# Ajay-Wong/seq2seq-attention-asr

Hardware: AMD Instinct MI355X
Metric: log-mel frames/sec fwd+bwd, Chorowski TIMIT baseline (higher is better)
Workload: dtype fp32; 1 GPU; BASELINE config 2: timit_chorowski_b32; model=timit/model_chorowski_baseline.lua, global_batch=32, utterances_per_gpu=32, seq_len=128, label_len=40, feat_dim=123, parallelism=dp1, allreduce=none, launch=hipGraph replay

## Files before the change

### seq2seq-attention-asr_amd/csrc/gru_persist.hip

```cpp
#include <algorithm>
#include <cstdlib>

#include "gru.h"
#include "gru_persist.h"
#include "handoff.h"
#include "skinny.h"

namespace s2s {

namespace {

struct PDir {
  const float* xp;
  long ldxp;
  const float* Wa;
  const float* Wb;
  float* y;
  long ldy;
  float* sv;
  const float* dy;
  long lddy;
  float* dA;
  long ldA;
  int reverse;
// ... 47 lines not shown
  x.ct = rem - x.d * q.ntn;
  return x;
}
__device__ __forceinline__ bool xunit_of(const XProj& q, int nd, int p, int nprod, int it, XUnit& x) {
  const int w = p + it * nprod;
  if (q.G == 0 || w < q.nsplit) {
    if (w >= q.nwork) return false;
    x = xunit(q, nd, w);
    return true;
  }
  const int nsp = q.nsplit > p ? (q.nsplit - p + nprod - 1) / nprod : 0;
  const int g = p / q.gsz, v = p - g * q.gsz + (it - nsp) * q.gsz;
  const int ncls = q.G / nd, i = v / q.ntn;
  x.sl = q.sB + i * ncls + g / nd;
  if (x.sl >= q.nslices) return false;
  x.d = g % nd;
  x.ct = v - i * q.ntn;
  x.part = 0;
  x.P = 1;
  x.item = -1;
  return true;
}
constexpr int kXpLds = 4 * 64 * 36 * 4;

struct WArgs {
  int nw;
  float* dW[2][3];
  float scale;
  const float* x;
  long ldx;
  int D, NP;
  float* part;
  unsigned* ticket;
  unsigned long long* stamps;
};

struct PArgs {
  XProj xq;
  int fused;
  PDir d[2];
  int B, L, H, MT, nwg;
  int nmem, nchains;
  int allow_local;
  unsigned* abort_word;
  unsigned* census;
  const int* len;
  char* next_sync;
  size_t next_prep;
  GruPackJobs pack;
  int ring;
  int stream_sweep;
  unsigned long long* stamps;
  unsigned long long* pstamps;
  int prefetch, prefetch_wg;
  unsigned* progress;
  WArgs wg;
};

#ifndef S2S_GRU_DIAG
#define S2S_GRU_DIAG 0
#endif
constexpr int kStampSlots = S2S_GRU_DIAG ? 16 : 8;
#define GRU_STAMP(ph)                                                                      \
  do {                                                                                     \
    if (a.stamps && threadIdx.x == 0)                                                      \
      a.stamps[((long)lw * a.L + s) * kStampSlots + (ph)] = __builtin_amdgcn_s_memrealtime(); \
  } while (0)
#define GRU_STAMP_V(ph, v)                                                                 \
  do {                                                                                     \
    if (a.stamps && threadIdx.x == 0) a.stamps[((long)lw * a.L + s) * kStampSlots + (ph)] = (v); \
  } while (0)
#if S2S_GRU_DIAG
template <int NC>
__device__ __forceinline__ bool sweep_sent_n(float4 (&a)[NC], __amdgpu_buffer_rsrc_t rs, long tbase, int rowt,
                                             int wave, int lane, unsigned* abort_word, unsigned& n) {
  const long lo = tbase + 4 * tile_lane(rowt, lane);
  unsigned spins = 0;
  while (true) {
    ++n;
    bool ok = true;
#pragma unroll
    for (int i = 0; i < NC; ++i) {
      const long off = lo + 4L * 256 * (wave + 4 * i);
      const uint4 p = __builtin_bit_cast(uint4, __builtin_amdgcn_raw_buffer_load_b128(rs, (int)off, 0, 16));
      ok = ok && p.x != kSent && p.y != kSent && p.z != kSent && p.w != kSent;
      a[i] = make_float4(__uint_as_float(p.x), __uint_as_float(p.y), __uint_as_float(p.z), __uint_as_float(p.w));
    }
    if (__all(ok)) return true;
    if (spin_give_up(spins, abort_word)) return false;
  }
}
#define SWEEP_SENT(slot_, ...) sweep_sent_n<NC>(__VA_ARGS__, npoll[slot_])
#else
#define SWEEP_SENT(slot_, ...) sweep_sent_tile<NC>(__VA_ARGS__)
#endif
std::atomic<unsigned long long*> g_gru_stamps[2] = {{nullptr}, {nullptr}};
std::atomic<unsigned long long*> g_gru_pstamps[2] = {{nullptr}, {nullptr}};
std::atomic<unsigned long long*> g_gru_wstamps{nullptr};
constexpr int kProdStampItems = 32;

__device__ __forceinline__ float reduce_or_abort(SkinnyRed& red, int* abort_lds, bool ok, floatx4 acc, int wave,
                                                 int lane, int tid, bool* aborted) {
  if (!ok) *abort_lds = 1;
  const float s = skinny_reduce(red, acc, wave, lane, tid);
  *aborted = *abort_lds != 0;
  return s;
}

template <bool NN, int D>
__device__ __forceinline__ void xproj_produce(const PArgs& a, float* lds, int p, int nprod) {
  const XProj& q = a.xq;
  const int tid = threadIdx.x, lane = tid & 63, wave = tid >> 6;
  const int nk = q.K / 32;
  __shared__ int last_part;
  const int nd = q.nd;
  if (tid >= 256) {
    XUnit x;
    for (int it = 0; xunit_of(q, nd, p, nprod, it, x); ++it) {
      const int nb = 1 + nk / x.P + (q.alpha ? 1 : 0);
      for (int i = 0; i < nb; ++i) __syncthreads();
      if (x.P == 1) {
        __syncthreads();
      } else {
        __syncthreads();
        __syncthreads();
        if (last_part) __syncthreads();
      }
    }
    return;
  }
  const int wy = wave >> 1, wx = wave & 1, li = lane & 31, lk = lane >> 5;
  const int B = a.B, L = a.L, H3 = q.ncd;
  constexpr int LDK = 36;
  float* As[2] = {lds, lds + 64 * LDK};
  float* Bs[2] = {lds + 128 * LDK, lds + 192 * LDK};
  int item = 0;
  XUnit xu;
  for (; xunit_of(q, nd, p, nprod, item, xu); ++item) {
    if (a.pstamps && tid == 0 && item < kProdStampItems)
      a.pstamps[((long)p * kProdStampItems + item) * 2] = __builtin_amdgcn_s_memrealtime();
    const int sl = xu.sl, d = xu.d, ct = xu.ct;
    const int nkp = nk / xu.P, kb = xu.part * nkp;
    const int rev = a.d[d].reverse ^ q.flip;
    const float* arow[2];
    const float* brow[2];
#pragma unroll
    for (int j = 0; j < 2; ++j) {
      const int r = (tid >> 3) + 32 * j, jt = r / B, b = r - jt * B, s = sl * q.tpt + jt;
      const bool aval = jt < q.tpt && s < L;
      const int t = rev ? L - 1 - s : s;
      arow[j] = q.x + (aval ? ((long)b * L + t) * q.ldx : 0);
      const int f = tid + 256 * j;
      brow[j] = NN ? q.W + (long)(f & 31) * q.ldw + d * H3 + ct * 64 + 4 * (f >> 5)
                   : q.W + (long)(d * H3 + ct * 64 + r) * q.ldw;
    }
    const int kq = 4 * (tid & 7);
    const long bstep = NN ? 32 * q.ldw : 32;
    floatx4 ra[D][2], rb[D][2];
    auto gload = [&](floatx4 (&xa)[2], floatx4 (&xb)[2], int kt) {
#pragma unroll
      for (int j = 0; j < 2; ++j) {
        xa[j] = *reinterpret_cast<const floatx4*>(arow[j] + 32 * kt + kq);
        xb[j] = *reinterpret_cast<const floatx4*>(brow[j] + kt * bstep + (NN ? 0 : kq));
      }
    };
    auto lstore = [&](const floatx4 (&xa)[2], const floatx4 (&xb)[2], int buf) {
      float* as = As[0] + buf * (64 * LDK);
      float* bs = Bs[0] + buf * (64 * LDK);
#pragma unroll
      for (int j = 0; j < 2; ++j) {
        const int f = tid + 256 * j;
        *reinterpret_cast<floatx4*>(as + (f >> 3) * LDK + 4 * (f & 7)) = xa[j];
        if (NN) {
          float* pb = bs + (4 * (f >> 5)) * LDK + (f & 31);
          pb[0] = xb[j][0];
          pb[LDK] = xb[j][1];
          pb[2 * LDK] = xb[j][2];
          pb[3 * LDK] = xb[j][3];
        } else {
          *reinterpret_cast<floatx4*>(bs + (f >> 3) * LDK + 4 * (f & 7)) = xb[j];
        }
      }
    };
    floatx16 acc;
#pragma unroll
    for (int r = 0; r < 16; ++r) acc[r] = 0.f;
    auto mma = [&](int buf, auto&& mid) {
      floatx4 av[4], bv[4];
      const float* pa = As[0] + buf * (64 * LDK) + (wy * 32 + li) * LDK + 16 * lk;
      const float* pb = Bs[0] + buf * (64 * LDK) + (wx * 32 + li) * LDK + 16 * lk;
#pragma unroll
// ... 110 lines not shown
        for (int i = 0; i < 4; ++i)
          pv[pp][i] = pp < xu.P ? __builtin_bit_cast(floatx4, __builtin_amdgcn_raw_buffer_load_b128(
                                                                  srs, ibase + pp * 16384 + 16 * i, 0, 16))
                                : floatx4{0.f, 0.f, 0.f, 0.f};
#pragma unroll
      for (int i = 0; i < 4; ++i)
#pragma unroll
        for (int e = 0; e < 4; ++e) {
          float v = pv[0][i][e] + pv[1][i][e];
          if (xu.P > 2) v = (v + pv[2][i][e]) + pv[3][i][e];
          acc[4 * i + e] = v;
        }
    }
#pragma unroll
    for (int r = 0; r < 16; ++r) {
      const int tr = wy * 32 + (r & 3) + 8 * (r >> 2) + 4 * lk, jt = tr / B, b = tr - jt * B, s = sl * q.tpt + jt;
      if (jt < q.tpt && s < L) {
        const int t = rev ? L - 1 - s : s;
        __hip_atomic_store(q.xp + ((long)b * L + t) * q.ldxp + col, 1.f * acc[r], __ATOMIC_RELAXED,
                           __HIP_MEMORY_SCOPE_AGENT);
      }
    }
    asm volatile("s_waitcnt vmcnt(0)" ::: "memory");
    __syncthreads();
    if (tid == 0) __hip_atomic_fetch_add(q.done + d * q.nslices + sl, 1u, __ATOMIC_RELAXED, __HIP_MEMORY_SCOPE_AGENT);
    if (a.pstamps && tid == 0 && item < kProdStampItems)
      a.pstamps[((long)p * kProdStampItems + item) * 2 + 1] = __builtin_amdgcn_s_memrealtime();
  }
}

template <bool NN>
__device__ __forceinline__ void xproj_produce_any(const PArgs& a, float* lds, int p, int nprod) {
  const int nk = a.xq.K / 32;
  if (nk % 4 == 0) xproj_produce<NN, 4>(a, lds, p, nprod);
  else if (nk % 3 == 0) xproj_produce<NN, 3>(a, lds, p, nprod);
  else if (nk % 2 == 0) xproj_produce<NN, 2>(a, lds, p, nprod);
  else xproj_produce<NN, 1>(a, lds, p, nprod);
}

__device__ __forceinline__ bool xproj_ready(const XProj& q, int d, int sl) {
  return __hip_atomic_load(q.done + d * q.nslices + sl, __ATOMIC_RELAXED, __HIP_MEMORY_SCOPE_AGENT) >=
         (unsigned)q.ntn;
}

__device__ __forceinline__ void xproj_wait(const XProj& q, int d, int need, int& ready, int lane, unsigned* abort_word) {
  unsigned spins = 0;
  while (need >= ready) {
    const int sl = ready + lane;
    const unsigned long long nr = __ballot(!(sl >= q.nslices || xproj_ready(q, d, sl)));
    const int upto = nr ? ready + (int)__builtin_ctzll(nr) : ready + 64;
    if (upto <= need && spin_give_up(spins, abort_word)) break;
    ready = upto;
  }
}

__device__ __forceinline__ void prep_next_sync(const PArgs& a, int sp, int nsp) {
  if (!a.next_sync) return;
  if (sp == 0 && threadIdx.x == 0) {
    unsigned* hdr = reinterpret_cast<unsigned*>(a.next_sync);
    const unsigned e = __hip_atomic_fetch_add(&g_s2s_epoch_ctr, 1u, __ATOMIC_RELAXED, __HIP_MEMORY_SCOPE_AGENT) + 1u;
    __hip_atomic_exchange(hdr + kEpochWord, e, __ATOMIC_RELAXED, __HIP_MEMORY_SCOPE_AGENT);
    rearm_abort_word(hdr);
  }
  const size_t n16 = (a.next_prep - 256) / 16;
  uint4* p = reinterpret_cast<uint4*>(a.next_sync + 256);
  for (size_t i = (size_t)sp * blockDim.x + threadIdx.x; i < n16; i += (size_t)nsp * blockDim.x)
    p[i] = make_uint4(0u, 0u, 0u, 0u);
  if (threadIdx.x == 0 && sp == 0 && (a.next_prep - 256) % 16) {
    unsigned* t = reinterpret_cast<unsigned*>(a.next_sync + 256 + n16 * 16);
    for (size_t i = 0; i < ((a.next_prep - 256) % 16) / 4; ++i) t[i] = 0u;
  }
}

constexpr int kRowRing = 4;
constexpr int kSentRing = 4;
__device__ __forceinline__ int sent_slot(const PArgs& a, int s) { return a.ring ? (s & (a.ring - 1)) : s; }
__device__ __forceinline__ void rearm_tile(float* role, const PArgs& a, int s, long tile, int lane) {
  const float4 sv = make_float4(__uint_as_float(kSent), __uint_as_float(kSent), __uint_as_float(kSent),
                                __uint_as_float(kSent));
  *reinterpret_cast<float4*>(role + (long)sent_slot(a, s) * a.MT * 16 * a.H + tile + 4 * lane) = sv;
}
constexpr int kFwdThreads = 320;
template <int NC>
__global__ __launch_bounds__(kFwdThreads) void gru_fwd_persist(PArgs a) {
  __shared__ SkinnyRed red;
  __shared__ int abort_lds, local_lds;
  __shared__ unsigned tb_lds;
  __shared__ __attribute__((aligned(16))) float hprev[16][16];
  __shared__ __attribute__((aligned(16))) float xring[kRowRing][2][256];
  __shared__ __attribute__((aligned(16))) float stg[2][3][256];
  extern __shared__ __attribute__((aligned(16))) float xlds[];
  const int H = a.H, B = a.B, L = a.L;
  const ChainSlot cs = chain_slot(a.nmem);
  if (cs.chain >= a.nchains) {
    const int gch = 8 * ((a.nchains + 7) / 8);
    const int sp = (cs.chain - a.nchains) * a.nmem + cs.member, nsp = (gch - a.nchains) * a.nmem;
    prep_next_sync(a, sp, nsp);
    if (a.fused) xproj_produce_any<false>(a, xlds, sp, nsp);
    for (int j = 0; j < a.pack.n; ++j)
      gru_pack_elems(a.pack.j[j], (long)sp * blockDim.x + threadIdx.x, (long)nsp * blockDim.x);
    return;
  }
  const int dir = cs.chain / a.MT, mt = cs.chain % a.MT;
  const PDir& g = a.d[dir];
  const int ncol = 2 * H / 16;
  const int c1 = cs.member;
  const int lw = dir * a.nwg + mt * ncol + c1;
  const bool isz = c1 < H / 16;
  const int tid = threadIdx.x, lane = tid & 63, wave = tid >> 6;
  const int b0 = mt * 16;
  if (tid == 0) abort_lds = 0;
  const unsigned tb = launch_tagbase(a.abort_word, &tb_lds);
  const bool loader = wave == 4;
  const long mytile = (long)mt * 16 * H + (long)(isz ? c1 : c1 - H / 16) * 256;
  if (!loader)
    rearm_rect((isz ? g.s0 : g.s1) + mytile, (long)a.MT * 16 * H, a.ring ? a.ring : L, 16, 0, 16, 0, 16);
  rearm_done();
  const bool loc = chain_is_local(a.census, cs.chain, a.nmem, c1, a.allow_local != 0, a.abort_word, &local_lds, tb);

  if (loader) {
    const int bl = b0 + (lane >> 2), col = c1 * 16 + 4 * (lane & 3);
    const bool lv = bl < B;
    const __amdgpu_buffer_rsrc_t xr = rsrc_of(g.xp);
    int xready = 0;
    auto issue = [&](int q, float4 (&r)[2]) {
      r[0] = r[1] = make_float4(0.f, 0.f, 0.f, 0.f);
      if (q >= L) return;
      if (a.fused) xproj_wait(a.xq, dir, q / a.xq.tpt, xready, lane, a.abort_word);
      if (!lv) return;
      const int t = g.reverse ? L - 1 - q : q;
      const long off = ((long)bl * L + t) * g.ldxp + col;
      if (a.fused) {
        r[0] = __builtin_bit_cast(float4, __builtin_amdgcn_raw_buffer_load_b128(xr, (int)(4 * off), 0, 16));
        if (isz)
          r[1] = __builtin_bit_cast(float4, __builtin_amdgcn_raw_buffer_load_b128(xr, (int)(4 * (off + 2 * H)), 0, 16));
      } else {
        r[0] = *reinterpret_cast<const float4*>(g.xp + off);
        if (isz) r[1] = *reinterpret_cast<const float4*>(g.xp + off + 2 * H);
      }
    };
    auto put = [&](int q, const float4 (&r)[2]) {
      *reinterpret_cast<float4*>(&xring[q % kRowRing][0][4 * lane]) = r[0];
      *reinterpret_cast<float4*>(&xring[q % kRowRing][1][4 * lane]) = r[1];
    };
    auto store = [&](int q) {
      if (!lv) return;
      const int t = g.reverse ? L - 1 - q : q;
      const long row = (long)bl * L + t;
      const float4 v0 = *reinterpret_cast<const float4*>(&stg[q & 1][0][4 * lane]);
      const float4 v1 = *reinterpret_cast<const float4*>(&stg[q & 1][1][4 * lane]);
      const float4 v2 = *reinterpret_cast<const float4*>(&stg[q & 1][2][4 * lane]);
      float* sv = g.sv + row * 5 * H;
      if (isz) {
        *reinterpret_cast<float4*>(sv + col) = v0;
        *reinterpret_cast<float4*>(sv + 2 * H + col) = v1;
        *reinterpret_cast<float4*>(g.y + row * g.ldy + col) = v2;
      } else {
        const int j = col - H;
        *reinterpret_cast<float4*>(sv + H + j) = v0;
        *reinterpret_cast<float4*>(sv + 3 * H + j) = v1;
        *reinterpret_cast<float4*>(sv + 4 * H + j) = v2;
      }
    };
    float4 ra[2], rb[2];
    issue(0, ra);
    issue(1, rb);
    put(0, ra);
    put(1, rb);
    issue(2, ra);
    __syncthreads();
    const bool ring = a.ring && loc;
    for (int s = 0; s < L; ++s) {
      if (ring) asm volatile("s_waitcnt vmcnt(0)" ::: "memory");
      __syncthreads();
      if (abort_lds) return;
      if (s > 0) store(s - 1);
      put(s + 2, ra);
      issue(s + 3, ra);
      if (ring) {
        if (isz && s >= 2) rearm_tile(g.s0, a, s - 2, mytile, lane);
        if (!isz && s >= 1) rearm_tile(g.s1, a, s - 1, mytile, lane);
      }
      if (!isz) continue;
      __syncthreads();
      if (abort_lds) return;
    }
    __syncthreads();
    store(L - 1);
    return;
  }

  float4 w1[NC], w2[NC];
  load_wfrag(w1, g.Wa + (long)(c1 * 16 + (lane & 15)) * H, wave, lane);
  if (isz) load_wfrag(w2, g.Wb + (long)(c1 * 16 + (lane & 15)) * H, wave, lane);

  const __amdgpu_buffer_rsrc_t hg = rsrc_of(g.g0), qg = rsrc_of(g.g1), hs = rsrc_of(g.s0), qs = rsrc_of(g.s1);
  const long slot = (long)B * H;
  const long slotS = (long)a.MT * 16 * H, tileS = (long)mt * 16 * H;
  const int rowt = min(b0 + (lane & 15), B - 1) - b0;
  const int br = min(b0 + (lane & 15), B - 1);
  const int ob = b0 + (tid >> 4), on = c1 * 16 + (tid & 15);
  const bool live = ob < B;
  const int lenb = (a.len && live) ? a.len[ob] : L;
  const int jt = c1 * 16 - H, wt = (jt % 64) / 16, it = jt / 64;
  float zreg = 0.f, hreg = 0.f;
  bool aborted = false;

  __syncthreads();
  for (int s = 0; s < L; ++s) {
    const int t = g.reverse ? L - 1 - s : s;
    floatx4 acc = {0.f, 0.f, 0.f, 0.f};
    bool ok = true;
    GRU_STAMP(0);
    if (s > 0) {
      float4 av[NC];
#if S2S_GRU_DIAG
      unsigned npoll[1] = {0};
#endif
      {
      if (loc) ok = SWEEP_SENT(0, av, hs, 4 * (sent_slot(a, s - 1) * slotS + tileS), rowt, wave, lane, a.abort_word);
      else ok = sweep_skinny<NC>(av, hg, 8 * (((s - 1) & 1) * slot + (long)br * H), tb + s, wave, lane, a.abort_word);
      GRU_STAMP(1);
#if S2S_GRU_DIAG
      GRU_STAMP_V(8, npoll[0]);
#endif
      acc = mfma_chunks<NC>(av, w1);
      }
      if (!isz && wave == wt) {
#pragma unroll
        for (int i = 0; i < NC; ++i)
          if (i == it) *reinterpret_cast<float4*>(&hprev[lane & 15][4 * (lane >> 4)]) = av[i];
// ... 315 lines not shown
  __shared__ int abort_lds, local_lds;
  __shared__ unsigned tb_lds;
  __shared__ __attribute__((aligned(16))) float rowq[kRowRing][5][256];
  extern __shared__ __attribute__((aligned(16))) float ylds[];
  const int H = a.H, B = a.B, L = a.L;
  const ChainSlot cs = chain_slot(a.nmem);
  const int gch = 8 * ((a.nchains + 7) / 8);
  if ((int)blockIdx.x >= chain_grid(a.nchains, a.nmem)) {
    const int pre = chain_grid(a.nchains, a.nmem) + (a.prefetch ? 8 * a.prefetch_wg : 0);
    if ((int)blockIdx.x < pre) {
      const int e = (int)blockIdx.x - chain_grid(a.nchains, a.nmem), c = e & 7, w = e >> 3;
      if (c < a.nchains) bptt_prefetch<NC>(a, c, w, a.prefetch_wg);
      return;
    }
    const int e = (int)blockIdx.x - pre, c = e & 7, w = e >> 3;
    if (c < a.nchains) bptt_wgrad<NC>(a, c, w, &tb_lds, &abort_lds);
    return;
  }
  if (cs.chain >= a.nchains) {
    const int sp = (cs.chain - a.nchains) * a.nmem + cs.member, nsp = (gch - a.nchains) * a.nmem;
    prep_next_sync(a, sp, nsp);
    if (a.fused) xproj_produce_any<true>(a, ylds, sp, nsp);
    return;
  }
  const int dir = cs.chain / a.MT, mt = cs.chain % a.MT;
  const PDir& g = a.d[dir];
  const int ncol = H / 16;
  const int c = cs.member;
  const int lw = dir * a.nwg + mt * ncol + c;
  const int tid = threadIdx.x, lane = tid & 63, wave = tid >> 6;
  const int b0 = mt * 16;
  if (a.stamps && tid == 0) a.stamps[((long)lw * L + L - 1) * 8 + 6] = __builtin_amdgcn_s_memrealtime();
  if (tid == 0) abort_lds = 0;
  const unsigned tb = launch_tagbase(a.abort_word, &tb_lds);
  const bool loader = wave == 4;
  const long mytile = (long)mt * 16 * H + (long)c * 256;
  if (!loader) {
    const long st = (long)a.MT * 16 * H;
    const int ns = a.ring ? a.ring : L;
    rearm_rect(g.s0 + mytile, st, ns, 16, 0, 16, 0, 16);
    rearm_rect(g.s1 + mytile, st, ns, 16, 0, 16, 0, 16);
    rearm_rect(g.s2 + mytile, st, ns, 16, 0, 16, 0, 16);
  }
  rearm_done();
  const bool loc = chain_is_local(a.census, cs.chain, a.nmem, c, a.allow_local != 0, a.abort_word, &local_lds, tb);
  if (a.stamps && tid == 0) a.stamps[((long)lw * L + L - 1) * 8 + 7] = __builtin_amdgcn_s_memrealtime();

  if (loader) {
    const int bl = b0 + (lane >> 2), u = c * 16 + 4 * (lane & 3);
    const bool lv = bl < B;
    const int lenl = (a.len && lv) ? a.len[bl] : L;
    const __amdgpu_buffer_rsrc_t dyr = rsrc_of(g.dy);
    int yready = 0;
    auto issue = [&](int q, float4 (&r)[5]) {
#pragma unroll
      for (int v = 0; v < 5; ++v) r[v] = make_float4(0.f, 0.f, 0.f, 0.f);
      if (q >= L) return;
      if (a.fused) xproj_wait(a.xq, dir, q / a.xq.tpt, yready, lane, a.abort_word);
      if (!lv) return;
#ifdef S2S_EXP_NOLOAD
      return;
#endif
      const int t = g.reverse ? q : L - 1 - q;
      const long row = (long)bl * L + t;
      const float* sv = g.sv + row * 5 * H + u;
#pragma unroll
      for (int v = 0; v < 4; ++v) r[v] = *reinterpret_cast<const float4*>(sv + v * H);
      if (t >= lenl) return;
      if (a.fused) {
        r[4] = __builtin_bit_cast(float4, __builtin_amdgcn_raw_buffer_load_b128(
                                              dyr, (int)(4 * (row * g.lddy + u)), 0, 16));
      } else {
        r[4] = *reinterpret_cast<const float4*>(g.dy + row * g.lddy + u);
      }
    };
    auto put = [&](int q, const float4 (&r)[5]) {
#pragma unroll
      for (int v = 0; v < 5; ++v) *reinterpret_cast<float4*>(&rowq[q % kRowRing][v][4 * lane]) = r[v];
    };
    float4 ra[5], rb[5];
    issue(0, ra);
    issue(1, rb);
    put(0, ra);
    put(1, rb);
    issue(2, ra);
    __syncthreads();
    const bool ring = a.ring && loc;
    unsigned* prog = a.progress ? a.progress + (long)cs.chain * a.nmem + c : nullptr;
    for (int p = 0; p < L; ++p) {
      __syncthreads();
      if (abort_lds) return;
      put(p + 2, ra);
      if (prog && lane == 0) __hip_atomic_store(prog, (unsigned)p, __ATOMIC_RELAXED, __HIP_MEMORY_SCOPE_WORKGROUP);
#ifndef S2S_EXP_LOADB
      issue(p + 3, ra);
#endif
      if (ring && p >= 1) {
        rearm_tile(g.s0, a, p - 1, mytile, lane);
        rearm_tile(g.s1, a, p - 1, mytile, lane);
        rearm_tile(g.s2, a, p - 1, mytile, lane);
      }
      asm volatile("s_waitcnt vmcnt(0)" ::: "memory");
      __syncthreads();
      if (abort_lds) return;
#ifdef S2S_EXP_LOADB
      issue(p + 3, ra);
#endif
    }
    if (a.wg.nw) {
      __syncthreads();
      if (lane == 0) __hip_atomic_store(prog, (unsigned)L + 3u, __ATOMIC_RELAXED, __HIP_MEMORY_SCOPE_AGENT);
    }
    return;
  }

  float4 wh[NC], wzr[2 * NC];
  load_wfrag(wh, g.Wa + (long)(c * 16 + (lane & 15)) * H, wave, lane);
  load_wfrag(wzr, g.Wb + (long)(c * 16 + (lane & 15)) * 2 * H, wave, lane);
  const __amdgpu_buffer_rsrc_t zg = rsrc_of(g.g0), rg = rsrc_of(g.g1), hg = rsrc_of(g.g2);
  const __amdgpu_buffer_rsrc_t zs = rsrc_of(g.s0), rs_ = rsrc_of(g.s1), hs = rsrc_of(g.s2);
  const long slot = (long)B * H;
  const int br = min(b0 + (lane & 15), B - 1);
  const long slotS = (long)a.MT * 16 * H, tileS = (long)mt * 16 * H;
  const int rowt = br - b0;
  const int ob = b0 + (tid >> 4), ok_ = c * 16 + (tid & 15);
  const bool live = ob < B;
  const int lenb = (a.len && live) ? a.len[ob] : L;
  float dhc = 0.f, dhp = 0.f;
  bool aborted = false;

  struct Row {
    float z, r, hh, hp, dy;
  };
  auto load_row = [&](int q) {
    const float(*r)[256] = rowq[q % kRowRing];
    return Row{r[0][tid], r[1][tid], r[2][tid], r[3][tid], r[4][tid]};
  };
  auto gate = [&](int t, const Row& v, float dh, int pn, bool pub) {
    const long row = (long)ob * L + t;
    const float daz = dh * (v.hh - v.hp) * (v.z * (1.0f - v.z));
    const float dah = (dh * v.z) * (1.0f - v.hh * v.hh);
    if (loc) {
      const long off = sent_slot(a, pn) * slotS + tile_off(ob, ok_, H);
      if (pub) {
        put_sent(g.s2 + off, dah);
        put_sent(g.s0 + off, daz);
      }
    } else {
      const long off = (pn & 1) * slot + (long)ob * H + ok_;
      put_granule_pair(g.g2, off, dah, tb + pn + 1, pub);
      put_granule_pair(g.g0, off, daz, tb + pn + 1, pub);
    }
#ifndef S2S_EXP_NODA
    if (pub) {
      g.dA[row * g.ldA + ok_] = daz;
      g.dA[row * g.ldA + 2 * H + ok_] = dah;
    }
#endif
  };

// ... 120 lines not shown
  const int nch = ndir * ((B + 15) / 16), nm = H / 16;
  const int nwg = std::max(1, std::min((int)g_bptt_prefetch_wg, nm));
  return g_bptt_prefetch > 0 && nch <= 8 && nm + nwg <= 32 && nm % nwg == 0 ? nwg : 0;
}
std::atomic<int> g_allow_local{1};
std::atomic<int> g_sent_ring{kSentRing};
std::atomic<int> g_stream_sweep{1};

template <int NC>
int launch_nc(hipStream_t st, const PArgs& a, bool excl_req, bool fwd) {
  const dim3 grid(chain_grid(a.nchains, a.nmem) + (!fwd && a.prefetch ? 8 * a.prefetch_wg : 0) +
                  (!fwd ? 8 * a.wg.nw : 0));
  const bool excl = excl_req && a.nchains <= 8 && a.nmem <= 32;
  const unsigned shm = excl ? kExclLds : (a.fused ? kXpLds : 0);
  if (fwd) {
    if (excl) S2S_CHECK_HIP(hipFuncSetAttribute(reinterpret_cast<const void*>(gru_fwd_persist<NC>),
                                                hipFuncAttributeMaxDynamicSharedMemorySize, kExclLds));
    S2S_TRY(check_resident(reinterpret_cast<const void*>(gru_fwd_persist<NC>), grid.x, kFwdThreads, shm,
                           "gru_fwd_persist"));
    hipLaunchKernelGGL(gru_fwd_persist<NC>, grid, dim3(kFwdThreads), shm, st, a);
  } else {
    if (excl) S2S_CHECK_HIP(hipFuncSetAttribute(reinterpret_cast<const void*>(gru_bwd_persist<NC>),
                                                hipFuncAttributeMaxDynamicSharedMemorySize, kExclLds));
    S2S_TRY(check_resident(reinterpret_cast<const void*>(gru_bwd_persist<NC>), grid.x, kBwdThreads, shm,
                           "gru_bwd_persist"));
    hipLaunchKernelGGL(gru_bwd_persist<NC>, grid, dim3(kBwdThreads), shm, st, a);
  }
  S2S_CHECK_HIP(hipGetLastError());
  return 0;
}

int launch(hipStream_t st, const PArgs& a, bool excl, bool fwd) {
  switch (a.H / 64) {
    case 1: return launch_nc<1>(st, a, excl, fwd);
    case 2: return launch_nc<2>(st, a, excl, fwd);
    case 4: return launch_nc<4>(st, a, excl, fwd);
    case 8: return launch_nc<8>(st, a, excl, fwd);
  }
  set_error("gru persistent: unsupported H");
  return 2;
}

}

std::atomic<int> g_fuse_xproj{1};

bool gru_persist_fused_xproj(int ndir, int B, int H, int Kx) {
  if (!g_fuse_xproj || B > 64 || Kx % 32 != 0 || H % 64 != 0) return false;
  const int MT = (B + 15) / 16, nchains = ndir * MT, nmem = 2 * H / 16;
  return chain_grid(nchains, nmem) - nchains * nmem >= 32;
}

std::atomic<int> g_xp_split{1};
std::atomic<int> g_fuse_dy{1};

bool gru_persist_fused_dy(int ndir, int B, int H, int K, long ldw, long lddy) {
  if (!g_fuse_xproj || !g_fuse_dy || B > 64 || K % 32 != 0 || H % 64 != 0 || ldw % 4 != 0 || lddy < (long)ndir * H) return false;
  const int MT = (B + 15) / 16, nchains = ndir * MT, nmem = H / 16;
  return chain_grid(nchains, nmem) - nchains * nmem >= 32;
}

bool gru_persist_wgrad_fits(int ndir, int B, int H, int D) {
  const int nch = ndir * ((B + 15) / 16), nm = H / 16, nw = 3 * H / 64;
  return H % 64 == 0 && D > 0 && nch <= 8 && nm + bptt_prefetch_wg(ndir, B, H) + nw <= 32 &&
         H + (D + 15) / 16 * 16 <= 4 * kWgCB * 16;
}

bool gru_persist_supported(int ndir, int B, int H) {
  if (!(H == 64 || H == 128 || H == 256 || H == 512)) return false;
  const int MT = (B + 15) / 16;
  return (2 * H / 16) * ((ndir * MT + 7) / 8) <= 64;
}

static size_t census_bytes(int B, int H) { return 4 * (size_t)(2 * ((B + 15) / 16)) * (2 * H / 16); }

static size_t xcount_words(int L) { return 2 * (size_t)L + kXpMaxSplitItems; }
static size_t prep_bytes(int B, int L, int H) {
  return 256 + 2 * 3 * 2 * sizeof(unsigned long long) * (size_t)B * H + census_bytes(B, H) + 4 * xcount_words(L) +
         census_bytes(B, H);
}
static size_t sent_offset(int B, int L, int H) { return (prep_bytes(B, L, H) + 255) / 256 * 256; }
static size_t sent_rows(int B) { return (size_t)(B + 15) / 16 * 16; }
static size_t slab_offset(int B, int L, int H) {
  return sent_offset(B, L, H) + 2 * 3 * sizeof(float) * (size_t)L * sent_rows(B) * H;
}
constexpr size_t kXpSlabBytes = (size_t)kXpMaxSplitItems * 4 * 4096 * sizeof(float);

size_t gru_persist_sync_bytes(int B, int L, int H) { return slab_offset(B, L, H) + kXpSlabBytes; }
size_t gru_persist_prep_bytes(int B, int L, int H) { return prep_bytes(B, L, H); }
bool gru_persist_can_prep_next(int ndir, int B, int H, bool fwd) {
  const int MT = (B + 15) / 16, nchains = ndir * MT, nmem = fwd ? 2 * H / 16 : H / 16;
  return chain_grid(nchains, nmem) > nchains * nmem;
}

static void xproj_split(XProj& q, int nd, int nprod) {
  q.sA = q.sB = 0;
  q.PA = q.PB = 1;
  q.nsplit = 0;
  const int nk = q.K / 32, per = nd * q.ntn;
  if (!g_xp_split || nk % 16 != 0 || per <= 0) return;
  const int sA = std::max(1, nprod / (per * 4));
  const int sB = std::min(q.nslices, sA + std::max(1, nprod / (per * 2)));
  if (sB > q.nslices || sB * per > kXpMaxSplitItems || sA >= sB) return;
  q.sA = sA; q.sB = sB; q.PA = 4; q.PB = 2;
  q.nwork = (sA * 4 + (sB - sA) * 2 + (q.nslices - sB)) * per;
  q.nsplit = (sA * 4 + (sB - sA) * 2) * per;
}

std::atomic<int> g_xp_group{1};

static void xproj_group(XProj& q, int nd, int nprod, int gsz) {
  q.G = 0;
  q.gsz = gsz;
  if (!g_xp_group || gsz <= 0 || nprod % gsz != 0) return;
  const int G = nprod / gsz;
  if (G < nd || G % nd != 0) return;
  q.G = G;
}

static void carve_granules(char* sync, int B, int L, int H, unsigned** abort_word, granule_t* (&g)[2][3],
                           float* (&sv)[2][3], unsigned** census, unsigned** xcount = nullptr) {
  *abort_word = reinterpret_cast<unsigned*>(sync);
  granule_t* p = reinterpret_cast<granule_t*>(sync + 256);
  for (int d = 0; d < 2; ++d)
    for (int k = 0; k < 3; ++k) {
      g[d][k] = p;
      p += 2L * B * H;
    }
  *census = reinterpret_cast<unsigned*>(p);
  if (xcount) *xcount = *census + census_bytes(B, H) / 4;
  float* q = reinterpret_cast<float*>(sync + sent_offset(B, L, H));
  for (int d = 0; d < 2; ++d)
    for (int k = 0; k < 3; ++k) {
      sv[d][k] = q;
      q += (long)L * sent_rows(B) * H;
    }
}

int gru_persist_fwd(hipStream_t st, const GruPersistFwd& f, void* sync) {
  PArgs a{};
  const int MT = (f.B + 15) / 16;
  granule_t* gr[2][3];
  float* sr[2][3];
  unsigned* xcount = nullptr;
  carve_granules(static_cast<char*>(sync), f.B, f.L, f.H, &a.abort_word, gr, sr, &a.census, &xcount);
  for (int d = 0; d < f.ndir; ++d)
    a.d[d] = PDir{f.xp[d], f.ldxp, f.Uzr[d], f.Uh[d], f.y[d], f.ldy, f.sv[d], nullptr, 0, nullptr, 0, f.reverse[d],
                  gr[d][0], gr[d][1], gr[d][2], sr[d][0], sr[d][1], sr[d][2]};
  a.len = f.len;
  a.B = f.B; a.L = f.L; a.H = f.H; a.MT = MT; a.nwg = (2 * f.H / 16) * MT;
  a.nmem = 2 * f.H / 16; a.nchains = f.ndir * MT; a.allow_local = g_allow_local;
  a.ring = f.L > kSentRing ? (int)g_sent_ring : 0;
  a.stream_sweep = g_stream_sweep;
  a.stamps = g_gru_stamps[0];
  a.pstamps = g_gru_pstamps[0];
  if (f.x) {
    XProj& q = a.xq;
    q.x = f.x; q.ldx = f.ldx; q.K = f.Kx; q.W = f.Wx; q.ldw = f.Kx; q.ncd = 3 * f.H; q.flip = 0;
    q.xp = const_cast<float*>(f.xp[0]); q.ldxp = f.ldxp;
    q.tpt = 64 / f.B;
    q.nslices = (f.L + q.tpt - 1) / q.tpt;
    q.ntn = 3 * f.H / 64;
    q.nd = f.ndir;
    q.nwork = q.nslices * f.ndir * q.ntn;
    q.done = xcount;
    q.sA = q.sB = 0; q.PA = q.PB = 1;
    a.fused = 1;
  }
  if (f.next_sync) {
    a.next_sync = static_cast<char*>(f.next_sync);
    a.next_prep = f.next_prep;
  }
  if (f.pack) a.pack = *f.pack;
  if (!f.prepared) S2S_TRY(launch_sync_prep(st, sync, prep_bytes(f.B, f.L, f.H), a.next_sync));
  const double xflops = f.x ? 2.0 * f.B * f.L * 3.0 * f.ndir * f.H * f.Kx : 0.0;
  const double xbytes = f.x ? 4.0 * ((double)f.B * f.L * f.Kx + 3.0 * f.ndir * f.H * f.Kx + 3.0 * f.ndir * f.B * f.L * f.H)
                            : 0.0;
  ProfScope ps(st, "gru_fwd_persist", 2.0 * f.ndir * f.B * f.L * 3.0 * f.H * f.H + xflops,
               4.0 * f.ndir * (3.0 * f.H * f.H + (double)f.B * f.L * (3 * f.H + 5 * f.H + f.H)) + xbytes);
  S2S_TRY(launch(st, a, f.excl != 0, true));
  void* r[1] = {sync};
  return launch_sync_harvest(st, r, 1, f.status);
}

int gru_persist_bwd(hipStream_t st, const GruPersistBwd& b, void* sync) {
  PArgs a{};
  const int MT = (b.B + 15) / 16;
  granule_t* gr[2][3];
  float* sr[2][3];
  unsigned* xcount = nullptr;
  carve_granules(static_cast<char*>(sync), b.B, b.L, b.H, &a.abort_word, gr, sr, &a.census, &xcount);
  {
    const int nwg = bptt_prefetch_wg(b.ndir, b.B, b.H);
    if (nwg) {
      a.prefetch = g_bptt_prefetch;
      a.prefetch_wg = nwg;
      a.progress = xcount + xcount_words(b.L);
    }
  }
  if (b.wgrad) {
    S2S_REQUIRE(gru_persist_wgrad_fits(b.ndir, b.B, b.H, b.wD) && b.wx && b.wpart,
                "gru persistent bwd: in-launch weight gradients do not fit this shape");
    WArgs& q = a.wg;
    q.nw = 3 * b.H / 64;
    for (int d = 0; d < 2; ++d)
      for (int g = 0; g < 3; ++g) q.dW[d][g] = b.wdW[d][g];
    q.scale = b.wscale;
    q.x = b.wx; q.ldx = b.wldx; q.D = b.wD; q.NP = b.H + (b.wD + 15) / 16 * 16;
    q.part = b.wpart;
    q.stamps = g_gru_wstamps;
    a.progress = xcount + xcount_words(b.L);
    q.ticket = a.progress + (long)b.ndir * MT * (b.H / 16);
  }
  for (int d = 0; d < b.ndir; ++d)
    a.d[d] = PDir{nullptr, 0, b.UhT[d], b.UzrT[d], nullptr, 0, b.sv[d], b.dy[d], b.lddy, b.dA[d], b.ldA,
                  b.reverse[d], gr[d][0], gr[d][1], gr[d][2], sr[d][0], sr[d][1], sr[d][2]};
  a.len = b.len;
  a.B = b.B; a.L = b.L; a.H = b.H; a.MT = MT; a.nwg = (b.H / 16) * MT;
  a.nmem = b.H / 16; a.nchains = b.ndir * MT; a.allow_local = g_allow_local;
  a.ring = b.L > kSentRing ? (int)g_sent_ring : 0;
  a.stream_sweep = g_stream_sweep;
  a.stamps = g_gru_stamps[1];
  a.pstamps = g_gru_pstamps[1];
  if (b.ydA) {
    XProj& q = a.xq;
    q.x = b.ydA; q.ldx = b.yldA; q.K = b.yK; q.W = b.yWx; q.ldw = b.yldw; q.ncd = b.H; q.flip = 1;
    q.xp = const_cast<float*>(b.dy[0]); q.ldxp = b.lddy;
    q.tpt = 64 / b.B;
    q.nslices = (b.L + q.tpt - 1) / q.tpt;
    q.ntn = b.H / 64;
    q.nd = b.ndir;
    q.nwork = q.nslices * b.ndir * q.ntn;
    q.done = xcount;
    q.alpha = b.yalpha; q.dc = b.ydc; q.T = b.yT;
    q.icnt = xcount + 2 * b.L;
    q.slab = reinterpret_cast<float*>(static_cast<char*>(sync) + slab_offset(b.B, b.L, b.H));
    const int gch = 8 * ((a.nchains + 7) / 8);
    xproj_split(q, b.ndir, (gch - a.nchains) * a.nmem);
    xproj_group(q, b.ndir, (gch - a.nchains) * a.nmem, a.nmem);
    a.fused = 1;
  }
  if (b.next_sync) {
    a.next_sync = static_cast<char*>(b.next_sync);
    a.next_prep = b.next_prep;
  }
  if (!b.prepared) S2S_TRY(launch_sync_prep(st, sync, prep_bytes(b.B, b.L, b.H), a.next_sync));
  if (b.prep_event) S2S_CHECK_HIP(hipEventRecord(b.prep_event, st));
  const double yflops = b.ydA ? 2.0 * b.B * b.L * (double)b.ndir * b.H * (b.yK + b.yT) : 0.0;
  const double ybytes = b.ydA ? 4.0 * ((double)b.B * b.L * b.yK + (double)b.yK * b.ndir * b.H +
                                       (double)b.B * b.yT * (b.L + b.ndir * b.H) + (double)b.B * b.L * b.ndir * b.H)
                              : 0.0;
  const double wflops = b.wgrad ? 2.0 * b.ndir * b.B * b.L * 3.0 * b.H * (b.H + b.wD) : 0.0;
  const double wbytes = b.wgrad ? 4.0 * ((double)b.B * b.L * (b.ndir * 3.0 * b.H + b.ndir * 2.0 * b.H + b.wD) +
                                         2.0 * b.ndir * 3.0 * b.H * (b.H + b.wD))
                                : 0.0;
  ProfScope ps(st, "gru_bwd_persist", 2.0 * b.ndir * b.B * b.L * 3.0 * b.H * b.H + yflops + wflops,
               4.0 * b.ndir * (3.0 * b.H * b.H + (double)b.B * b.L * (5 * b.H + b.H + 3 * b.H)) + ybytes + wbytes);
  S2S_TRY(launch(st, a, b.excl != 0, false));
  void* r[1] = {sync};
  return launch_sync_harvest(st, r, 1, b.status);
}

__global__ __launch_bounds__(64) void handoff_timeout_probe(char* sync) {
  unsigned* hdr = reinterpret_cast<unsigned*>(sync);
  const granule_t* g = reinterpret_cast<const granule_t*>(sync + 256);
  unsigned spins = 0;
  while (true) {
    const granule_t x = __hip_atomic_load(g + threadIdx.x, __ATOMIC_RELAXED, __HIP_MEMORY_SCOPE_AGENT);
    if (__all((unsigned)(x >> 32) == 0xfffffffeu)) break;
    if (spin_give_up(spins, hdr, 4096u)) break;
  }
}
int handoff_timeout_probe_launch(hipStream_t st, void* sync, unsigned* status) {
  S2S_TRY(launch_sync_prep(st, sync, 256 + 64 * sizeof(granule_t)));
  hipLaunchKernelGGL(handoff_timeout_probe, dim3(1), dim3(64), 0, st, static_cast<char*>(sync));
  S2S_CHECK_HIP(hipGetLastError());
// ... 60 lines not shown
  float acc = 0.f;
  int k = threadIdx.x;
  while (__builtin_amdgcn_s_memrealtime() - t0 < ticks) {
    k = (k * 7 + 13) % n;
    acc += hog[k];
    __builtin_amdgcn_s_sleep(8);
  }
  if (acc == -1.f) out[blockIdx.x] = acc;
}
int lds_hog_launch(hipStream_t st, int nwg, int lds_bytes, double usec, float* out) {
  S2S_REQUIRE(nwg > 0 && nwg <= 4096 && lds_bytes >= 1024 && lds_bytes <= 160 * 1024 && usec > 0 && usec < 1e6,
              "lds hog: bad arguments");
  S2S_CHECK_HIP(hipFuncSetAttribute(reinterpret_cast<const void*>(lds_hog_kernel),
                                    hipFuncAttributeMaxDynamicSharedMemorySize, lds_bytes));
  hipLaunchKernelGGL(lds_hog_kernel, dim3(nwg), dim3(256), lds_bytes, st, out, lds_bytes / 4,
                     (unsigned long long)(usec * 100.0));
  S2S_CHECK_HIP(hipGetLastError());
  return 0;
}

__global__ __launch_bounds__(64) void clock_probe_kernel(unsigned long long* out, int n, unsigned long long period) {
  if (threadIdx.x != 0) return;
  unsigned long long* o = out + 2ull * n * blockIdx.x;
  for (int i = 0; i < n; ++i) {
    const unsigned long long r = __builtin_amdgcn_s_memrealtime();
    const unsigned long long c = __builtin_amdgcn_s_memtime();
    o[2 * i] = r;
    o[2 * i + 1] = c;
    while (__builtin_amdgcn_s_memrealtime() - r < period) __builtin_amdgcn_s_sleep(2);
  }
}
int clock_probe_launch(hipStream_t st, int nwg, int n, int period, unsigned long long* out) {
  S2S_REQUIRE(nwg > 0 && nwg <= 64 && n > 0 && n <= (1 << 20) && period > 0 && (double)n * period < 2e8,
              "clock probe: bad arguments");
  hipLaunchKernelGGL(clock_probe_kernel, dim3(nwg), dim3(64), 0, st, out, n, (unsigned long long)period);
  S2S_CHECK_HIP(hipGetLastError());
  return 0;
}

}

extern "C" int s2s_debug_clock_probe(void* stream, int nwg, int n, int period, unsigned long long* out) {
  return s2s::clock_probe_launch(static_cast<hipStream_t>(stream), nwg, n, period, out);
}

extern "C" int s2s_debug_lds_hog(void* stream, int nwg, int lds_bytes, double usec, float* out) {
  return s2s::lds_hog_launch(static_cast<hipStream_t>(stream), nwg, lds_bytes, usec, out);
}

extern "C" void s2s_debug_gru_local(int allow) { s2s::g_allow_local = allow; }
extern "C" void s2s_debug_gru_fused_xproj(int on) { s2s::g_fuse_xproj = on; }
extern "C" void s2s_debug_gru_fused_dy(int on) { s2s::g_fuse_dy = on; }
extern "C" void s2s_debug_gru_xp_split(int on) { s2s::g_xp_split = on; }
extern "C" void s2s_debug_gru_xp_group(int on) { s2s::g_xp_group = on; }
extern "C" void s2s_debug_bptt_prefetch(int wg, int lookahead) {
  s2s::g_bptt_prefetch_wg = wg;
  s2s::g_bptt_prefetch = lookahead;
}
extern "C" void s2s_debug_gru_stream_sweep(int on) { s2s::g_stream_sweep = on; }
extern "C" void s2s_debug_gru_ring(int on) { s2s::g_sent_ring = on ? s2s::kSentRing : 0; }
extern "C" void s2s_debug_gru_stamps(void* fwd, void* bwd) {
  s2s::g_gru_stamps[0] = static_cast<unsigned long long*>(fwd);
  s2s::g_gru_stamps[1] = static_cast<unsigned long long*>(bwd);
}
extern "C" void s2s_debug_gru_wg_stamps(void* p) { s2s::g_gru_wstamps = static_cast<unsigned long long*>(p); }
extern "C" void s2s_debug_gru_prod_stamps(void* fwd, void* bwd) {
  s2s::g_gru_pstamps[0] = static_cast<unsigned long long*>(fwd);
  s2s::g_gru_pstamps[1] = static_cast<unsigned long long*>(bwd);
}
```

Baseline: 1.391 million frames/s.

## Poll producer readiness to schedule backward row prefetch, retune xproj split and grouping

After: 1.401 million frames/s, median of 6. About the same (+0.7%).

```diff
diff --git a/seq2seq-attention-asr_amd/csrc/gru_persist.hip b/seq2seq-attention-asr_amd/csrc/gru_persist.hip
--- a/seq2seq-attention-asr_amd/csrc/gru_persist.hip
+++ b/seq2seq-attention-asr_amd/csrc/gru_persist.hip
@@ -123,6 +123,7 @@
   int stream_sweep;
   unsigned long long* stamps;
   unsigned long long* pstamps;
+  unsigned xp_pause;
   int prefetch, prefetch_wg;
   unsigned* progress;
   WArgs wg;
@@ -208,6 +209,10 @@
   int item = 0;
   XUnit xu;
   for (; xunit_of(q, nd, p, nprod, item, xu); ++item) {
+    if (a.xp_pause) {
+      const unsigned long long t0 = __builtin_amdgcn_s_memrealtime();
+      while (__builtin_amdgcn_s_memrealtime() - t0 < a.xp_pause) __builtin_amdgcn_s_sleep(8);
+    }
     if (a.pstamps && tid == 0 && item < kProdStampItems)
       a.pstamps[((long)p * kProdStampItems + item) * 2] = __builtin_amdgcn_s_memrealtime();
     const int sl = xu.sl, d = xu.d, ct = xu.ct;
@@ -424,6 +429,65 @@
     if (upto <= need && spin_give_up(spins, abort_word)) break;
     ready = upto;
   }
+}
+__device__ __forceinline__ bool xproj_poll(const XProj& q, int d, int need, int& ready, int lane) {
+  if (need >= ready) {
+    const int sl = ready + lane;
+    const unsigned long long nr = __ballot(!(sl >= q.nslices || xproj_ready(q, d, sl)));
+    ready = nr ? ready + (int)__builtin_ctzll(nr) : ready + 64;
+  }
+  return need < ready;
+}
+
+struct RowSched {
+  int nx = 0;
+  bool held = false;
+};
+template <class Regs, class Wait, class Poll, class Load, class Put>
+__device__ __forceinline__ void rows_start(RowSched& rs, int L, Regs& ra, Regs& rb, Wait&& wait, Poll&& poll,
+                                           Load&& load, Put&& put) {
+  wait(0);
+  const bool r1 = 1 < L && poll(1), r2 = r1 && 2 < L && poll(2);
+  load(0, ra);
+  if (r1) load(1, rb);
+  put(0, ra);
+  if (r1) put(1, rb);
+  if (r2) load(2, ra);
+  rs.nx = 1 + (r1 ? 1 : 0) + (r2 ? 1 : 0);
+  rs.held = r2;
+}
+__device__ __forceinline__ void vm_drain() {
+  __builtin_amdgcn_s_waitcnt(0x0f70);
+  asm volatile("" ::: "memory");
+}
+template <class Regs, class Put>
+__device__ __forceinline__ void rows_put(RowSched& rs, Regs& ra, Put&& put) {
+  if (rs.held) {
+    put(rs.nx - 1, ra);
+    rs.held = false;
+  }
+}
+template <class Regs, class Wait, class Poll, class Load, class Put>
+__device__ __forceinline__ void rows_advance(RowSched& rs, int p, int L, Regs& ra, Regs& rb, Wait&& wait,
+                                             Poll&& poll, Load&& load, Put&& put) {
+  if (rs.nx == p + 1 && rs.nx < L) {
+    wait(rs.nx);
+    load(rs.nx, rb);
+    put(rs.nx, rb);
+    ++rs.nx;
+  }
+  bool late = false;
+  if (rs.nx == p + 2 && rs.nx < L && poll(rs.nx)) {
+    load(rs.nx, rb);
+    late = true;
+    ++rs.nx;
+  }
+  if (rs.nx == p + 3 && rs.nx < L && poll(rs.nx)) {
+    load(rs.nx, ra);
+    rs.held = true;
+    ++rs.nx;
+  }
+  if (late) put(p + 2, rb);
 }
 
 __device__ __forceinline__ void prep_next_sync(const PArgs& a, int sp, int nsp) {
@@ -495,10 +559,14 @@
     const bool lv = bl < B;
     const __amdgpu_buffer_rsrc_t xr = rsrc_of(g.xp);
     int xready = 0;
+    auto wait = [&](int q) {
+      if (a.fused) xproj_wait(a.xq, dir, q / a.xq.tpt, xready, lane, a.abort_word);
+    };
+#ifdef S2S_EXP_FWD_ROWSCHED
+    auto poll = [&](int q) { return !a.fused || xproj_poll(a.xq, dir, q / a.xq.tpt, xready, lane); };
+#endif
     auto issue = [&](int q, float4 (&r)[2]) {
       r[0] = r[1] = make_float4(0.f, 0.f, 0.f, 0.f);
-      if (q >= L) return;
-      if (a.fused) xproj_wait(a.xq, dir, q / a.xq.tpt, xready, lane, a.abort_word);
       if (!lv) return;
       const int t = g.reverse ? L - 1 - q : q;
       const long off = ((long)bl * L + t) * g.ldxp + col;
@@ -535,20 +603,38 @@
       }
     };
     float4 ra[2], rb[2];
-    issue(0, ra);
-    issue(1, rb);
+#ifdef S2S_EXP_FWD_ROWSCHED
+    RowSched rows;
+    rows_start(rows, L, ra, rb, wait, poll, issue, put);
+#else
+    auto issue_w = [&](int q, float4 (&r)[2]) {
+      r[0] = r[1] = make_float4(0.f, 0.f, 0.f, 0.f);
+      if (q >= L) return;
+      wait(q);
+      issue(q, r);
+    };
+    issue_w(0, ra);
+    issue_w(1, rb);
     put(0, ra);
     put(1, rb);
-    issue(2, ra);
+    issue_w(2, ra);
+#endif
     __syncthreads();
     const bool ring = a.ring && loc;
     for (int s = 0; s < L; ++s) {
       if (ring) asm volatile("s_waitcnt vmcnt(0)" ::: "memory");
       __syncthreads();
       if (abort_lds) return;
+#ifdef S2S_EXP_FWD_ROWSCHED
+      vm_drain();
+      rows_put(rows, ra, put);
+      if (s > 0) store(s - 1);
+      rows_advance(rows, s, L, ra, rb, wait, poll, issue, put);
+#else
       if (s > 0) store(s - 1);
       put(s + 2, ra);
-      issue(s + 3, ra);
+      issue_w(s + 3, ra);
+#endif
       if (ring) {
         if (isz && s >= 2) rearm_tile(g.s0, a, s - 2, mytile, lane);
         if (!isz && s >= 1) rearm_tile(g.s1, a, s - 1, mytile, lane);
@@ -970,11 +1056,13 @@
     const int lenl = (a.len && lv) ? a.len[bl] : L;
     const __amdgpu_buffer_rsrc_t dyr = rsrc_of(g.dy);
     int yready = 0;
+    auto wait = [&](int q) {
+      if (a.fused) xproj_wait(a.xq, dir, q / a.xq.tpt, yready, lane, a.abort_word);
+    };
+    auto poll = [&](int q) { return !a.fused || xproj_poll(a.xq, dir, q / a.xq.tpt, yready, lane); };
     auto issue = [&](int q, float4 (&r)[5]) {
 #pragma unroll
       for (int v = 0; v < 5; ++v) r[v] = make_float4(0.f, 0.f, 0.f, 0.f);
-      if (q >= L) return;
-      if (a.fused) xproj_wait(a.xq, dir, q / a.xq.tpt, yready, lane, a.abort_word);
       if (!lv) return;
 #ifdef S2S_EXP_NOLOAD
       return;
@@ -997,33 +1085,26 @@
       for (int v = 0; v < 5; ++v) *reinterpret_cast<float4*>(&rowq[q % kRowRing][v][4 * lane]) = r[v];
     };
     float4 ra[5], rb[5];
-    issue(0, ra);
-    issue(1, rb);
-    put(0, ra);
-    put(1, rb);
-    issue(2, ra);
+    RowSched rows;
+    rows_start(rows, L, ra, rb, wait, poll, issue, put);
     __syncthreads();
     const bool ring = a.ring && loc;
     unsigned* prog = a.progress ? a.progress + (long)cs.chain * a.nmem + c : nullptr;
     for (int p = 0; p < L; ++p) {
       __syncthreads();
       if (abort_lds) return;
-      put(p + 2, ra);
+      vm_drain();
+      rows_put(rows, ra, put);
       if (prog && lane == 0) __hip_atomic_store(prog, (unsigned)p, __ATOMIC_RELAXED, __HIP_MEMORY_SCOPE_WORKGROUP);
-#ifndef S2S_EXP_LOADB
-      issue(p + 3, ra);
-#endif
+      rows_advance(rows, p, L, ra, rb, wait, poll, issue, put);
       if (ring && p >= 1) {
         rearm_tile(g.s0, a, p - 1, mytile, lane);
         rearm_tile(g.s1, a, p - 1, mytile, lane);
         rearm_tile(g.s2, a, p - 1, mytile, lane);
       }
-      asm volatile("s_waitcnt vmcnt(0)" ::: "memory");
+      vm_drain();
       __syncthreads();
       if (abort_lds) return;
-#ifdef S2S_EXP_LOADB
-      issue(p + 3, ra);
-#endif
     }
     if (a.wg.nw) {
       __syncthreads();
@@ -1250,6 +1331,7 @@
 }
 
 std::atomic<int> g_xp_split{1};
+std::atomic<unsigned> g_xp_pause{0};
 std::atomic<int> g_fuse_dy{1};
 
 bool gru_persist_fused_dy(int ndir, int B, int H, int K, long ldw, long lddy) {
@@ -1298,14 +1380,14 @@
   const int nk = q.K / 32, per = nd * q.ntn;
   if (!g_xp_split || nk % 16 != 0 || per <= 0) return;
   const int sA = std::max(1, nprod / (per * 4));
-  const int sB = std::min(q.nslices, sA + std::max(1, nprod / (per * 2)));
+  const int sB = std::min(q.nslices, sA + std::max(1, nprod / (per * 4)));
   if (sB > q.nslices || sB * per > kXpMaxSplitItems || sA >= sB) return;
   q.sA = sA; q.sB = sB; q.PA = 4; q.PB = 2;
   q.nwork = (sA * 4 + (sB - sA) * 2 + (q.nslices - sB)) * per;
   q.nsplit = (sA * 4 + (sB - sA) * 2) * per;
 }
 
-std::atomic<int> g_xp_group{1};
+std::atomic<int> g_xp_group{0};
 
 static void xproj_group(XProj& q, int nd, int nprod, int gsz) {
   q.G = 0;
@@ -1352,6 +1434,7 @@
   a.stream_sweep = g_stream_sweep;
   a.stamps = g_gru_stamps[0];
   a.pstamps = g_gru_pstamps[0];
+  a.xp_pause = g_xp_pause;
   if (f.x) {
     XProj& q = a.xq;
     q.x = f.x; q.ldx = f.ldx; q.K = f.Kx; q.W = f.Wx; q.ldw = f.Kx; q.ncd = 3 * f.H; q.flip = 0;
@@ -1420,6 +1503,7 @@
   a.stream_sweep = g_stream_sweep;
   a.stamps = g_gru_stamps[1];
   a.pstamps = g_gru_pstamps[1];
+  a.xp_pause = g_xp_pause;
   if (b.ydA) {
     XProj& q = a.xq;
     q.x = b.ydA; q.ldx = b.yldA; q.K = b.yK; q.W = b.yWx; q.ldw = b.yldw; q.ncd = b.H; q.flip = 1;
@@ -1586,6 +1670,7 @@
 extern "C" void s2s_debug_gru_fused_xproj(int on) { s2s::g_fuse_xproj = on; }
 extern "C" void s2s_debug_gru_fused_dy(int on) { s2s::g_fuse_dy = on; }
 extern "C" void s2s_debug_gru_xp_split(int on) { s2s::g_xp_split = on; }
+extern "C" void s2s_debug_gru_prod_pause(int usec) { s2s::g_xp_pause = 100u * (unsigned)std::min(std::max(usec, 0), 50); }
 extern "C" void s2s_debug_gru_xp_group(int on) { s2s::g_xp_group = on; }
 extern "C" void s2s_debug_bptt_prefetch(int wg, int lookahead) {
   s2s::g_bptt_prefetch_wg = wg;
```
